# Chemical118/TREW

Hardware: NVIDIA B200
Metric: Gbases/s for trew short 5 32 at 1/2/4/8 B200; % of HBM roofline (higher is better)
Workload: dtype u64

## Files before the change

trew_b200/csrc/exact_thread.cuh:

```cuda
#pragma once
#include <stdint.h>

#if defined(__CUDACC__)
#define ET_HD __host__ __device__ __forceinline__
#define ET_FN __host__ __device__ __noinline__
#else
#define ET_HD inline
#define ET_FN inline
#endif
#if defined(__CUDA_ARCH__)
#define ET_UNROLL _Pragma("unroll")
#define ET_NO_UNROLL _Pragma("unroll 1")
#else
#define ET_UNROLL
#define ET_NO_UNROLL
#endif

namespace trew {
namespace et {

typedef uint32_t u32;
typedef uint64_t u64;
typedef unsigned __int128 u128;

// ... 13 lines not shown
    static constexpr int KW = (int)(sizeof(K) / 4);
    static constexpr int CT = W_CKEY + KW * kClsCap, WORDS = CT + kClsCap;
};
constexpr int kWorkWords = Lay<u64>::WORDS;

struct Mem {
    u32* base; int stride;
    ET_HD u32& operator[](int i) const { return base[i * stride]; }
};

ET_HD int popc(u32 x) {
#if defined(__CUDA_ARCH__)
    return __popc(x);
#else
    return __builtin_popcount(x);
#endif
}
ET_HD int ffs1(u32 x) {
#if defined(__CUDA_ARCH__)
    return __ffs(x) - 1;
#else
    return __builtin_ctz(x);
#endif
}
ET_HD u32 fshr(u32 lo, u32 hi, int sh) {
#if defined(__CUDA_ARCH__)
    return __funnelshift_r(lo, hi, sh);
#else
    sh &= 31;
    return sh ? (lo >> sh) | (hi << (32 - sh)) : lo;
#endif
}
ET_HD u32 brev32(u32 x) {
#if defined(__CUDA_ARCH__)
    return __brev(x);
#else
    x = ((x >> 1) & 0x55555555u) | ((x & 0x55555555u) << 1);
    x = ((x >> 2) & 0x33333333u) | ((x & 0x33333333u) << 2);
    x = ((x >> 4) & 0x0f0f0f0fu) | ((x & 0x0f0f0f0fu) << 4);
    x = ((x >> 8) & 0x00ff00ffu) | ((x & 0x00ff00ffu) << 8);
    return (x >> 16) | (x << 16);
#endif
}
ET_HD u32 lowmask(int bits) { return bits >= 32 ? 0xffffffffu : (bits <= 0 ? 0u : ((1u << bits) - 1u)); }
ET_HD u32 pxor32(u32 x) { x ^= x << 1; x ^= x << 2; x ^= x << 4; x ^= x << 8; x ^= x << 16; return x; }
ET_HD u64 spread(u32 x) {
    u64 v = x;
    v = (v | (v << 16)) & 0x0000FFFF0000FFFFULL;
    v = (v | (v << 8)) & 0x00FF00FF00FF00FFULL;
    v = (v | (v << 4)) & 0x0F0F0F0F0F0F0F0FULL;
    v = (v | (v << 2)) & 0x3333333333333333ULL;
    v = (v | (v << 1)) & 0x5555555555555555ULL;
    return v;
}

ET_FN u64 canon64(u64 w, int k) {
    const int sh = 2 * (k - 1);
    if (k <= 16) {
        u32 b = (u32)w, c = (u32)w;
        for (int r = 1; r < k; r++) { c = ((c & 3u) << sh) | (c >> 2); b = c < b ? c : b; }
        return b;
    }
    u64 best = w, cur = w;
    for (int r = 1; r < k; r++) { cur = ((cur & 3ULL) << sh) | (cur >> 2); best = cur < best ? cur : best; }
    return best;
}
ET_FN u128 canon128(u128 w, int k) {
    const int sh = 2 * (k - 1);
    u128 best = w, cur = w;
    for (int r = 1; r < k; r++) { cur = ((cur & 3) << sh) | (cur >> 2); best = cur < best ? cur : best; }
    return best;
}
ET_HD u64 canon(u64 w, int k) { return canon64(w, k); }
ET_HD u128 canon(u128 w, int k) { return k <= 32 ? (u128)canon64((u64)w, k) : canon128(w, k); }
ET_HD u64 crc(u64 w, int k) {
    const u32 lo = brev32((u32)w), hi = brev32((u32)(w >> 32));
    u64 x = ((u64)lo << 32) | hi;
    x = ((x >> 1) & 0x5555555555555555ULL) | ((x & 0x5555555555555555ULL) << 1);
    return canon64(~x >> (64 - 2 * k), k);
}
ET_HD u128 crc(u128 w, int k) {
    if (k <= 32) return (u128)crc((u64)w, k);
    u128 r = 0;
    for (int i = 0; i < k; i++) { r = (r << 2) | (3 - (w & 3)); w >>= 2; }
    return canon128(r, k);
}
ET_HD bool homo(u64 w, int k) {
    return k <= 1 || ((w ^ (w >> 2)) & ((1ULL << (2 * (k - 1))) - 1ULL)) == 0;
}
ET_HD bool homo(u128 w, int k) {
    return k <= 1 || ((w ^ (w >> 2)) & ((((u128)1) << (2 * (k - 1))) - 1)) == 0;
}

template <class K>
struct ClsSpill {
    K key[kClsSpill];
    unsigned short tot[kClsSpill], last[kClsSpill];
};

template <class K>
ET_HD K cls_key(Mem m, int q) {
    K v = 0;
    for (int i = Lay<K>::KW - 1; i >= 0; i--) v = (v << 16 << 16) | (K)m[W_CKEY + Lay<K>::KW * q + i];
    return v;
}
template <class K>
ET_HD void cls_put(Mem m, int q, K key) {
    for (int i = 0; i < Lay<K>::KW; i++) { m[W_CKEY + Lay<K>::KW * q + i] = (u32)key; key = key >> 16 >> 16; }
}

ET_HD u32 shr_plane(Mem m, int base, int j, int k) {
    if (k < 32) return fshr(m[base + j], m[base + j + 1], k);
    if (k == 32) return m[base + j + 1];
    if (k < 64) return fshr(m[base + j + 1], m[base + j + 2], k - 32);
    return m[base + j + 2];
}

ET_HD u64 raw_kmer(Mem m, int j, int b, int k, u64& hk, u64& lk, u64) {
    const u32 km = lowmask(k);
    const u32 h = fshr(m[W_H + j], m[W_H + j + 1], b) & km, l = fshr(m[W_L + j], m[W_L + j + 1], b) & km;
    hk = h; lk = l;
    return (spread(brev32(h) >> (32 - k)) << 1) | spread(brev32(l) >> (32 - k));
}
ET_HD u128 raw_kmer(Mem m, int j, int b, int k, u64& hk, u64& lk, u128) {
    if (k <= 32) return (u128)raw_kmer(m, j, b, k, hk, lk, (u64)0);
    const u64 km = k >= 64 ? ~0ULL : ((1ULL << k) - 1ULL);
    hk = ((u64)fshr(m[W_H + j], m[W_H + j + 1], b) | ((u64)fshr(m[W_H + j + 1], m[W_H + j + 2], b) << 32)) & km;
    lk = ((u64)fshr(m[W_L + j], m[W_L + j + 1], b) | ((u64)fshr(m[W_L + j + 1], m[W_L + j + 2], b) << 32)) & km;
    const u64 hr = (((u64)brev32((u32)hk) << 32) | brev32((u32)(hk >> 32))) >> (64 - k);
    const u64 lr = (((u64)brev32((u32)lk) << 32) | brev32((u32)(lk >> 32))) >> (64 - k);
    const u64 lo = (spread((u32)hr) << 1) | spread((u32)lr), hi = (spread((u32)(hr >> 32)) << 1) | spread((u32)(lr >> 32));
    return ((u128)hi << 64) | lo;
}

ET_HD u32 run_starts(Mem m, int j) {
    return m[W_WV + j] & ~((m[W_LINK + j] << 1) | (j ? m[W_LINK + j - 1] >> 31 : 0u));
}
ET_FN int prepare_runs(Mem m, int nw, int k) {
    for (int j = 0; j < nw; j++) {
        const u32 hs = shr_plane(m, W_H, j, k), ls = shr_plane(m, W_L, j, k);
        const u32 eq = ~((hs ^ m[W_H + j]) | (ls ^ m[W_L + j]));
        const u32 wvj = m[W_WV + j];
        const u32 nxt = (wvj >> 1) | (j + 1 < nw ? m[W_WV + j + 1] << 31 : 0u);
        m[W_LINK + j] = eq & wvj & nxt;
    }
    int runs = 0;
    for (int j = 0; j < nw; j++) runs += popc(run_starts(m, j));
    return runs;
}

constexpr int kMemo = 4;
#if defined(ET_MEMO_STATS) && !defined(__CUDA_ARCH__)
inline long memo_runs = 0, memo_hits = 0;
#define ET_MEMO_COUNT(hit) (memo_runs++, memo_hits += (hit) >= 0)
#else
#define ET_MEMO_COUNT(hit) ((void)0)
#endif
template <class K>
ET_FN int classify_runs(Mem m, int runs, int k, ClsSpill<K>& x, bool approx, int T = 0, int need_min = 0) {
    int n = 0, ord = 0, j = 0, best = 0;
    const int slack = T - need_min;
    K mraw[kMemo];
    u32 mcls = 0;
    int nm = 0;
    u32 wvj = m[W_WV], rr = run_starts(m, 0);
    for (int r = 0; r < runs; r++) {
        while (!rr) { ord += popc(wvj); j++; rr = run_starts(m, j); wvj = m[W_WV + j]; }
        {
            const int b = ffs1(rr);
            rr &= rr - 1;
            const u32 c0 = (u32)(ord + popc(wvj & ((1u << b) - 1u)));
            int jj = j;
            u32 z = ~m[W_LINK + j] & (0xffffffffu << b);
            while (!z) { jj++; z = ~m[W_LINK + jj]; }
            const u32 cnt = (u32)(32 * (jj - j) + ffs1(z) - b + 1);
            u64 hk, lk;
            const K raw = raw_kmer(m, j, b, k, hk, lk, (K)0);
            const u32 last = c0 + cnt - 1u;
            int hit = -1;
            if (!approx) {
ET_UNROLL
                for (int e = 0; e < kMemo; e++) hit = e < nm && mraw[e] == raw ? (int)((mcls >> (8 * e)) & 0xffu) : hit;
            }
            if (!approx) ET_MEMO_COUNT(hit);
            u32 tot = cnt;
            if (hit >= kClsCap) {
                const int s = hit - kClsCap;
                tot = x.tot[s] + cnt; x.tot[s] = (unsigned short)tot; x.last[s] = (unsigned short)last;
            } else if (hit >= 0) {
                const u32 ct = (m[Lay<K>::CT + hit] & 0xffff0000u) + (cnt << 16);
                m[Lay<K>::CT + hit] = ct | last;
                tot = ct >> 16;
            } else {
                K key;
                if (approx) key = (K)((u32)(popc((u32)hk) + popc((u32)(hk >> 32))) | ((u32)(popc((u32)lk) + popc((u32)(lk >> 32))) << 8) |
                                      ((u32)(popc((u32)(hk & lk)) + popc((u32)((hk & lk) >> 32))) << 16));
                else key = canon(raw, k);
                int q = 0;
                const int nq = n < kClsCap ? n : kClsCap;
                while (q < nq && cls_key<K>(m, q) != key) q++;
                if (q < nq) {
                    const u32 ct = (m[Lay<K>::CT + q] & 0xffff0000u) + (cnt << 16);
                    m[Lay<K>::CT + q] = ct | last;
                    tot = ct >> 16;
                } else if (n < kClsCap) {
                    cls_put<K>(m, n, key); m[Lay<K>::CT + n] = (cnt << 16) | last;
                    n++;
                } else {
                    int s = 0;
                    while (s < n - kClsCap && x.key[s] != key) s++;
                    if (s < n - kClsCap) { tot = x.tot[s] + cnt; x.tot[s] = (unsigned short)tot; x.last[s] = (unsigned short)last; }
                    else { x.key[s] = key; x.tot[s] = (unsigned short)cnt; x.last[s] = (unsigned short)last; n++; }
                    q = kClsCap + s;
                }
                if (!approx && nm < kMemo) {
ET_UNROLL
                    for (int e = 0; e < kMemo; e++) if (e == nm) mraw[e] = raw;
                    mcls |= (u32)q << (8 * nm);
                    nm++;
                }
            }
            if (need_min > 0) {
                best = (int)tot > best ? (int)tot : best;
                if ((int)last + 1 - best > slack) return -1;
            }
        }
    }
    return n;
}

template <class K>
ET_FN int cls_max(Mem m, int n, const ClsSpill<K>& x, K& S) {
    u32 best = 0;
    S = 0;
    for (int q = 0; q < n && q < kClsCap; q++) {
        const u32 ct = m[Lay<K>::CT + q];
        const u32 score = ((ct >> 16) << 10) | (1023u - (ct & 0xffffu));
        if (score > best) { best = score; S = cls_key<K>(m, q); }
    }
    for (int q = 0; q < n - kClsCap; q++) {
        const u32 score = ((u32)x.tot[q] << 10) | (1023u - x.last[q]);
        if (score > best) { best = score; S = x.key[q]; }
    }
    return (int)(best >> 10);
}

ET_HD bool need_pass(const unsigned short* thr, u32 need, int M, int T) {
    const u32 mm = need & 0xffffu, t = need >> 16;
    return M >= (int)thr[T] && (t == 0u || (u32)M * t >= mm * (u32)T);
}

ET_HD int min_accept(const unsigned short* thr, u32 need, int T) {
    const u32 mm = need & 0xffffu, t = need >> 16;
    const int a = (int)thr[T], b = t ? (int)((mm * (u32)T + t - 1u) / t) : 0;
    return a > b ? a : b;
}

ET_HD void shrink_valid(Mem m, int nw) {
    for (int j = 0; j < nw; j++) m[W_WV + j] &= (m[W_WV + j] >> 1) | (j + 1 < nw ? m[W_WV + j + 1] << 31 : 0u);
}

template <int NW>
ET_HD void shrink_valid(u32 (&wv)[NW]) {
ET_UNROLL
    for (int j = 0; j < NW; j++) wv[j] &= (wv[j] >> 1) | (j + 1 < NW ? wv[j + 1] << 31 : 0u);
}
template <int S, int NW>
ET_HD void sig_counts(const u32 (&ph)[NW + 2], const u32 (&pl)[NW + 2], const u32 (&wv)[NW], int k, int& cH, int& cL, int& c11) {
ET_UNROLL
    for (int j = 0; j < NW; j++) {
        const u32 dh = (fshr(ph[S + j], S + j + 1 < NW + 2 ? ph[S + j + 1] : 0u, k) ^ ph[j]) & wv[j];
        const u32 dl = (fshr(pl[S + j], S + j + 1 < NW + 2 ? pl[S + j + 1] : 0u, k) ^ pl[j]) & wv[j];
        cH += popc(dh); cL += popc(dl); c11 += popc(dh & dl);
    }
}

template <class K> struct PeriodSet { typedef u64 T; };
template <> struct PeriodSet<u64> { typedef u32 T; };

template <class K, int NW>
ET_HD u32 scan_periods(Mem m, int len, int kmin, int kmax, const unsigned short* thr_low, const unsigned short* thr_high, ClsSpill<K>& x,
                       K (&S)[2]) {
    const int nw = (len + 31) >> 5;
    u32 ph[NW + 2], pl[NW + 2], wv[NW];
    {
        u32 ch = 0, cl = 0, tph = 0, tpl = 0;
ET_UNROLL
        for (int j = 0; j <= NW; j++) {
            const u32 ih = pxor32(m[W_H + j]) ^ ch, il = pxor32(m[W_L + j]) ^ cl;
            ph[j] = (ih << 1) | tph; pl[j] = (il << 1) | tpl;
            tph = ih >> 31; tpl = il >> 31;
            ch = 0u - tph; cl = 0u - tpl;
        }
        ph[NW + 1] = 0u; pl[NW + 1] = 0u;
    }
ET_UNROLL
    for (int j = 0; j < NW; j++) wv[j] = j < nw ? m[W_V + j] : 0u;
    for (int t = 1; t < kmin; t++) shrink_valid<NW>(wv);
    typedef typename PeriodSet<K>::T Set;
    Set blockedL = 0, blockedH = 0;
    u32 needL = 0, needH = 0;
    u32 res = 0;
ET_NO_UNROLL
    for (int k = kmin; k <= kmax; k++, shrink_valid<NW>(wv)) {
        const bool blkL = (bool)((blockedL >> (k - 1)) & 1u), blkH = (bool)((blockedH >> (k - 1)) & 1u);
        int T = 0, cH = 0, cL = 0, c11 = 0;
ET_UNROLL
        for (int j = 0; j < NW; j++) T += popc(wv[j]);
        if (T == 0) break;
        if (blkL && blkH) continue;
        if (k < 32) sig_counts<0, NW>(ph, pl, wv, k, cH, cL, c11);
        else if constexpr (sizeof(K) == 8) sig_counts<1, NW>(ph, pl, wv, k, cH, cL, c11);
        else if (k < 64) sig_counts<1, NW>(ph, pl, wv, k, cH, cL, c11);
        else sig_counts<2, NW>(ph, pl, wv, k, cH, cL, c11);
        const int c10 = cH - c11, c01 = cL - c11, c00 = T - cH - cL + c11;
        int U = c00 > c01 ? c00 : c01;
        U = U > c10 ? U : c10;
        U = U > c11 ? U : c11;
        if (!((!blkL && need_pass(thr_low, needL, U, T)) || (!blkH && need_pass(thr_high, needH, U, T)))) continue;
        K Sk;
ET_UNROLL
        for (int j = 0; j < NW; j++) m[W_WV + j] = wv[j];
        const int runs = prepare_runs(m, nw, k);
        int need_min = 1 << 20;
        if (!blkL) need_min = min_accept(thr_low, needL, T);
        if (!blkH) { const int a = min_accept(thr_high, needH, T); need_min = a < need_min ? a : need_min; }
        if (runs > 3 && T <= kApproxMaxWindows) {
            const int na = classify_runs(m, runs, k, x, true, T, need_min);
            if (na < 0) continue;
            const int Mu = cls_max(m, na, x, Sk);
            if (!((!blkL && need_pass(thr_low, needL, Mu, T)) || (!blkH && need_pass(thr_high, needH, Mu, T)))) continue;
        }
        const int n = classify_runs(m, runs, k, x, false, T, need_min);
        if (n < 0) continue;
        const int M = cls_max(m, n, x, Sk);
        if (homo(Sk, k)) continue;
        const bool accL = !blkL && need_pass(thr_low, needL, M, T), accH = !blkH && need_pass(thr_high, needH, M, T);
        if (accL || accH) {
            Set mm = 0;
            for (int j = k; j <= kmax; j += k) mm |= ((Set)1) << (j - 1);
            const u32 need = (u32)M | ((u32)T << 16);
            if (accL) { res = (res & 0xffu) | ((u32)k << 8); needL = need; blockedL |= mm; S[1] = Sk; }
            if (accH) { res = (res & 0xff00u) | (u32)k; needH = need; blockedH |= mm; S[0] = Sk; }
        }
    }
    return res;
}
template <class K>
ET_FN u32 scan_window(Mem m, int len, int kmin, int kmax, const unsigned short* thr_low, const unsigned short* thr_high, ClsSpill<K>& x,
                      K (&S)[2]) {
    S[0] = S[1] = 0;
    if (kmax > len) kmax = len;
    if (kmax < kmin) return 0u;
    if (len <= 96) return scan_periods<K, 3>(m, len, kmin, kmax, thr_low, thr_high, x, S);
    return scan_periods<K, kReadWords>(m, len, kmin, kmax, thr_low, thr_high, x, S);
}

enum { T_F = 0, T_B = 2, T_O = 4 };

template <class K, class Emit>
ET_HD void emit_window_classes(Mem m, int len, int k, int table, bool folded, ClsSpill<K>& x, Emit& emit);

template <class K, class Load, class Emit>
ET_HD bool route_short_thread(Mem m, int n, u32 pm, int min_mer, int max_mer, const unsigned short* thr_low,
                              const unsigned short* thr_high, Load& load, Emit& emit) {
    if (n < 2 * min_mer) return true;
    if (max_mer > (int)(4 * sizeof(K)) || n > kMaxRead) return false;
    const int kmax = n / 4 < max_mer ? n / 4 : max_mer;
    const int llen = n / 2, rlen = (n + 1) / 2, roff = n - rlen;
    ClsSpill<K> x;
    u32 L = 0, R = 0;
    K S[2];
    const bool halves = n >= 4 * min_mer;
    for (u32 todo = halves ? pm & 3u : 0u; todo != 0u; todo &= todo - 1u) {
        const bool right = (todo & 1u) == 0u;
        const int len = right ? rlen : llen;
        load(0, right ? roff : 0, len);
        const u32 r = scan_window(m, len, min_mer, kmax, thr_low, thr_high, x, S);
        if (right) R = r; else L = r;
    }
    if (4 * max_mer > n) {
        const bool hc0 = ((L | R) & 0xffu) == 0u, hc1 = ((L | R) >> 8) == 0u;
        const u32 wbit = halves ? 4u : 1u;
        if ((hc0 || hc1) && (pm & wbit)) {
            const int lo = n / 4 + 1 > min_mer ? n / 4 + 1 : min_mer, hi = n / 2 < max_mer ? n / 2 : max_mer;
            load(0, 0, n);
            const u32 W = scan_window(m, n, lo, hi, thr_low, thr_high, x, S);
            for (int c = 0; c < 2; c++) {
                const int k = (int)((W >> (8 * c)) & 0xffu);
                if ((c == 0 ? hc0 : hc1) && k) emit_window_classes(m, n, k, T_O + c, false, x, emit);
            }
        }
    }
    if ((L | R) == 0u) return true;
    int cur_win = -1, cur_k = 0, ncls = 0, T = 0;
    for (int c = 0; c < 2; c++) {
        const int Lc = (int)((L >> (8 * c)) & 0xffu), Rc = (int)((R >> (8 * c)) & 0xffu);
        int win, k, table;
        if (Lc > 0 && Lc == Rc) { win = 2; k = Lc; table = T_O + c; }
        else if (Lc > 0) { win = 0; k = Lc; table = T_F + c; }
        else if (Rc > 0) { win = 1; k = Rc; table = T_B + c; }
        else continue;
        if (win != cur_win || k != cur_k) {
            const int off = win == 1 ? roff : 0, len = win == 2 ? n : (win == 0 ? llen : rlen), nw = (len + 31) >> 5;
            load(0, off, len);
            for (int j = 0; j < nw; j++) m[W_WV + j] = m[W_V + j];
            for (int t = 1; t < k; t++) shrink_valid(m, nw);
            T = 0;
            for (int j = 0; j < nw; j++) T += popc(m[W_WV + j]);
            ncls = 0;
            if (T) ncls = classify_runs(m, prepare_runs(m, nw, k), k, x, false);
            cur_win = win; cur_k = k;
        }
        if (T == 0) continue;
        const bool target = win == 2;
        if (target) {
            K S;
            const int M = cls_max(m, ncls, x, S);
            if (homo(S, k) || M < (int)(c == 0 ? thr_high : thr_low)[T]) continue;
        }
        for (int q = 0; q < ncls; q++) {
            K key = q < kClsCap ? cls_key<K>(m, q) : x.key[q - kClsCap];
            const u64 cnt = q < kClsCap ? (u64)(m[Lay<K>::CT + q] >> 16) : (u64)x.tot[q - kClsCap];
            if (target) { const K t = crc(key, k); key = t < key ? t : key; }
            emit(table, k, key, cnt);
        }
    }
    return true;
}

template <class K, class Emit>
ET_HD void emit_window_classes(Mem m, int len, int k, int table, bool folded, ClsSpill<K>& x, Emit& emit) {
    const int nw = (len + 31) >> 5;
    for (int j = 0; j < nw; j++) m[W_WV + j] = m[W_V + j];
    for (int t = 1; t < k; t++) shrink_valid(m, nw);
    int T = 0;
    for (int j = 0; j < nw; j++) T += popc(m[W_WV + j]);
    if (T == 0) return;
    const int ncls = classify_runs(m, prepare_runs(m, nw, k), k, x, false);
    for (int q = 0; q < ncls; q++) {
        K key = q < kClsCap ? cls_key<K>(m, q) : x.key[q - kClsCap];
        const u64 cnt = q < kClsCap ? (u64)(m[Lay<K>::CT + q] >> 16) : (u64)x.tot[q - kClsCap];
        if (folded) { const K t = crc(key, k); key = t < key ? t : key; }
        emit(table, k, key, cnt);
    }
}

template <class K, class Load, class Emit>
ET_HD bool route_pair_thread(Mem m, int n1, int n2, int min_mer, int max_mer, const unsigned short* thr_low,
                             const unsigned short* thr_high, Load& load, Emit& emit) {
    const int n = n1 < n2 ? n1 : n2;
    if (n < 2 * min_mer) return true;
    if (max_mer > (int)(4 * sizeof(K)) || n1 > kMaxRead || n2 > kMaxRead || 4 * max_mer > n) return false;
    const int kmax = n / 4 < max_mer ? n / 4 : max_mer;
    const int soff[5] = {0, 0, n1 - (n1 + 1) / 2, n2 - (n2 + 1) / 2, 0};
    const int slen[5] = {0, n1 / 2, (n1 + 1) / 2, (n2 + 1) / 2, n2 / 2};
    ClsSpill<K> x;
    u32 res[5] = {0, 0, 0, 0, 0};
    K S[5][2];
    bool have[5] = {false, false, false, false, false};
    auto window = [&](int t) { load(t <= 2 ? 0 : 1, soff[t], slen[t]); };
    auto scan = [&](int t) {
        if (have[t]) return;
        window(t);
        res[t] = scan_window(m, slen[t], min_mer, kmax, thr_low, thr_high, x, S[t]);
        have[t] = true;
    };
    int pseg[2][8], ptmp[2][8], np[2] = {0, 0};
    int si[2] = {1, 1}, km[2] = {0, 0};
    bool ended[2] = {false, false};
    K ks[2] = {0, 0};
    for (int ti = 1; ti <= 4 && !(ended[0] && ended[1]); ti++) {
        scan(ti);
        for (int c = 0; c < 2; c++) {
            const int k = (int)((res[ti] >> (8 * c)) & 0xffu);
            if (!ended[c] && k) { pseg[c][np[c]] = ti; ptmp[c][np[c]] = ti <= 2 ? 0 : 1; np[c]++; }
            bool ok = !ended[c] && k > 0;
            if (ok && ti != 1) {
                const K ds = ti > 2 ? crc(S[ti][c], k) : S[ti][c];
                ok = km[c] == k && ks[c] == ds;
            }
            if (ok) { si[c]++; km[c] = k; if (ti == 1) ks[c] = S[ti][c]; }
            else ended[c] = true;
        }
    }
    for (int c = 0; c < 2; c++) {
        if (si[c] == 5) {
            for (int e = 0; e < np[c]; e++) {
                const int sg = pseg[c][e];
                window(sg);
                emit_window_classes(m, slen[sg], (int)((res[sg] >> (8 * c)) & 0xffu), T_O + c, true, x, emit);
            }
        }
    }
    if (si[0] <= 4 || si[1] <= 4) {
        int sj[2] = {4, 4};
        km[0] = km[1] = 0; ended[0] = ended[1] = false;
        for (int tj = 4; tj >= 1 && !(ended[0] && ended[1]); tj--) {
            scan(tj);
            for (int c = 0; c < 2; c++) {
                const int k = (int)((res[tj] >> (8 * c)) & 0xffu);
                if (!ended[c] && k) { pseg[c][np[c]] = tj; ptmp[c][np[c]] = tj <= 2 ? 1 : 0; np[c]++; }
                bool ok = sj[c] >= si[c] && !ended[c] && k > 0;
                if (ok && tj != 4) {
                    const K ds = tj <= 2 ? crc(S[tj][c], k) : S[tj][c];
                    ok = km[c] == k && ks[c] == ds;
                }
                if (ok) { sj[c]--; km[c] = k; if (tj == 4) ks[c] = S[tj][c]; }
                else ended[c] = true;
            }
        }
    }
    for (int c = 0; c < 2; c++) {
        if (si[c] <= 4) {
            for (int e = 0; e < np[c]; e++) {
                const int sg = pseg[c][e];
                window(sg);
                emit_window_classes(m, slen[sg], (int)((res[sg] >> (8 * c)) & 0xffu), (ptmp[c][e] == 0 ? T_F : T_B) + c, false, x, emit);
            }
        }
    }
    return true;
}


struct LongGeom {
    int n, SL, snum, mid, bonus;
    ET_HD LongGeom(int n_, int SL_) : n(n_), SL(SL_), snum(n_ / SL_), mid((n_ / SL_ + 1) / 2), bonus(n_ % SL_) {}
    ET_HD int start(int t) const { return (t - 1) * SL + (t > mid ? bonus : 0); }
    ET_HD int len(int t) const { return SL + (t == mid ? bonus : 0); }
};

template <class Load>
ET_HD u32 long_slice_stats(Mem m, const LongGeom& g, int t, int min_mer, int max_mer, const unsigned short* thr_low,
                           const unsigned short* thr_high, Load& load, ClsSpill<u64>& x) {
    const int len = g.len(t);
    load(0, g.start(t), len);
    u64 S[2];
    return scan_window(m, len, min_mer, max_mer, thr_low, thr_high, x, S);
}

struct LongTask { unsigned short slice; unsigned char k, table_folded; };

template <class Stat, class Task>
ET_HD bool long_walk(const LongGeom& g, Stat& stat, Task& task) {
    const int snum = g.snum;
    const bool mid_ok = g.len(g.mid) <= kMaxRead;
    for (int pass = mid_ok ? 1 : 0; pass < 2; pass++) {
        int si[2] = {1, 1}, km[2] = {0, 0};
        bool ended[2] = {false, false};
        int nf = 0;
        for (int ti = 1; ti <= snum && !(ended[0] && ended[1]); ti++) {
            if (pass == 0 && ti == g.mid) return false;
            const u32 r = stat(ti);
            for (int c = 0; c < 2; c++) {
                const int k = (int)((r >> (8 * c)) & 0xffu);
                if (!ended[c] && k > 0 && (ti == 1 || km[c] == k)) { si[c]++; km[c] = k; }
                else ended[c] = true;
            }
            nf = ti;
        }
        if (pass == 1) {
            bool en[2] = {false, false};
            int kk[2] = {0, 0};
            const bool full[2] = {si[0] == snum + 1, si[1] == snum + 1};
            for (int ti = 1; ti <= nf; ti++) {
                const u32 r = stat(ti);
                for (int c = 0; c < 2; c++) {
                    const int k = (int)((r >> (8 * c)) & 0xffu);
                    if (!en[c] && k) task(LongTask{(unsigned short)ti, (unsigned char)k, (unsigned char)(((full[c] ? T_O : T_F) + c) | (full[c] ? 8 : 0))});
                    if (!en[c] && k > 0 && (ti == 1 || kk[c] == k)) kk[c] = k;
                    else en[c] = true;
                }
            }
        }
        if (si[0] <= snum || si[1] <= snum) {
            int sj[2] = {snum, snum};
            km[0] = km[1] = 0; ended[0] = ended[1] = false;
            for (int tj = snum; tj >= 1 && !(ended[0] && ended[1]); tj--) {
                if (pass == 0 && tj == g.mid) return false;
// ... 23 lines not shown
```

trew_b200/csrc/scan_kernels.cu:

```cuda
#include "scan_kernels.cuh"
#include "exact_thread.cuh"

#include <cstdio>

namespace trew {

typedef unsigned int u32;
typedef unsigned long long u64;
typedef unsigned __int128 u128;


__device__ __forceinline__ u32 lane_id() { return threadIdx.x & 31; }

__device__ __forceinline__ u32 low_mask(int bits) {
    return bits >= 32 ? 0xffffffffu : ((1u << bits) - 1u);
}

__device__ __forceinline__ u32 prefix_xor32(u32 x) {
    x ^= x << 1; x ^= x << 2; x ^= x << 4; x ^= x << 8; x ^= x << 16;
    return x;
}

__device__ __forceinline__ u64 mix64(u64 x) {
    x ^= x >> 33; x *= 0xff51afd7ed558ccdULL; x ^= x >> 33; x *= 0xc4ceb9fe1a85ec53ULL; x ^= x >> 33;
// ... 1440 lines not shown
                if (!have[tj]) { sr[tj] = scan_stats(ws, b, spos[tj], slen[tj], MINM, kmax, cfg); have[tj] = true; }
                int k[2] = {sr[tj].th, sr[tj].tl};
                u64 slo[2] = {sr[tj].sh_lo, sr[tj].sl_lo}, shi[2] = {sr[tj].sh_hi, sr[tj].sl_hi};
#pragma unroll
                for (int c = 0; c < 2; c++) {
                    if (!ended[c] && k[c]) { pseg[c][np[c]] = tj; ptmp[c][np[c]] = tj <= 2 ? 1 : 0; np[c]++; }
                    bool ok = sj[c] >= si[c] && !ended[c] && k[c] > 0;
                    if (ok && tj != 4) {
                        u64 dlo = slo[c], dhi = shi[c];
                        if (tj <= 2) crc_pair(dlo, dhi, k[c]);
                        ok = km[c] == k[c] && ks_lo[c] == dlo && ks_hi[c] == dhi;
                    }
                    if (ok) { sj[c]--; km[c] = k[c]; if (tj == 4) { ks_lo[c] = slo[c]; ks_hi[c] = shi[c]; } }
                    else ended[c] = true;
                }
            }
        }
#pragma unroll
        for (int c = 0; c < 2; c++) {
            if (si[c] <= 4) {
                for (int e = 0; e < np[c]; e++) {
                    int sg = pseg[c][e];
                    emit_window(tr, ws, b, spos[sg], slen[sg], c == 0 ? sr[sg].th : sr[sg].tl,
                                (ptmp[c][e] == 0 ? T_F : T_B) + c, false);
                }
            }
        }
    }
    if (4 * MAXM > n && (lef[0] == 0 || lef[1] == 0 || km[0] == 0 || km[1] == 0)) {
        int lo = max(n / 4 + 1, MINM), hi = min(n / 2, MAXM);
        ScanRes l, r; l.th = l.tl = r.th = r.tl = 0; l.sh_lo = l.sh_hi = l.sl_lo = l.sl_hi = 0; r = l;
        if (lef[0] == 0 || lef[1] == 0) l = scan_stats(ws, b, a0, n1, lo, hi, cfg);
        if (km[0] == 0 || km[1] == 0) r = scan_stats(ws, b, a1, n2, lo, hi, cfg);
        int ltk[2] = {l.th, l.tl}, rtk[2] = {r.th, r.tl};
        u64 llo[2] = {l.sh_lo, l.sl_lo}, lhi[2] = {l.sh_hi, l.sl_hi}, rlo[2] = {r.sh_lo, r.sl_lo}, rhi[2] = {r.sh_hi, r.sl_hi};
#pragma unroll
        for (int c = 0; c < 2; c++) {
            bool el = lef[c] == 0 && ltk[c] > 0, er = km[c] == 0 && rtk[c] > 0;
            bool both = lef[c] == 0 && km[c] == 0 && ltk[c] == rtk[c] && ltk[c] > 0;
            if (both) {
                u64 dlo = rlo[c], dhi = rhi[c];
                crc_pair(dlo, dhi, rtk[c]);
                both = llo[c] == dlo && lhi[c] == dhi;
            }
            if (both) {
                if (el) emit_window(tr, ws, b, a0, n1, ltk[c], T_O + c, true);
                if (er) emit_window(tr, ws, b, a1, n2, rtk[c], T_O + c, true);
            }
            if (el) emit_window(tr, ws, b, a0, n1, ltk[c], T_F + c, false);
            if (er) emit_window(tr, ws, b, a1, n2, rtk[c], T_F + c, false);
        }
    }
}

__device__ void route_long(const DevCfg& cfg, TableRef tr, WS ws, const DevBatch& b, u32 u, unsigned char* scratch) {
    const int MINM = cfg.min_mer, MAXM = cfg.max_mer, SL = cfg.slice_len;
    u32 b0 = __ldg(b.bit_off + u);
    int n = (int)(__ldg(b.bit_off + u + 1) - b0);
    if (n < SL) return;
    int snum = n / SL, mid = (snum + 1) / 2, bonus = n % SL;
    auto s_start = [&](int t) { return (u32)((t - 1) * SL + (t > mid ? bonus : 0)); };
    auto s_len = [&](int t) { return SL + (t == mid ? bonus : 0); };
    int si[2] = {1, 1}, km[2] = {0, 0}; bool ended[2] = {false, false};
    int nf = 0;
    for (int ti = 1; ti <= snum && !(ended[0] && ended[1]); ti++) {
        ScanRes sr = scan_stats(ws, b, b0 + s_start(ti), s_len(ti), MINM, MAXM, cfg);
        if (ws.lane == 0) { scratch[2 * (ti - 1)] = (unsigned char)sr.th; scratch[2 * (ti - 1) + 1] = (unsigned char)sr.tl; }
        int k[2] = {sr.th, sr.tl};
#pragma unroll
        for (int c = 0; c < 2; c++) {
            if (!ended[c] && k[c] > 0 && (ti == 1 || km[c] == k[c])) { si[c]++; km[c] = k[c]; }
            else ended[c] = true;
        }
        nf = ti;
    }
    __syncwarp();
    {
        bool en[2] = {false, false}; int kk[2] = {0, 0};
        bool full[2] = {si[0] == snum + 1, si[1] == snum + 1};
        for (int ti = 1; ti <= nf; ti++) {
            int k[2] = {scratch[2 * (ti - 1)], scratch[2 * (ti - 1) + 1]};
#pragma unroll
            for (int c = 0; c < 2; c++) {
                if (!en[c] && k[c]) emit_window(tr, ws, b, b0 + s_start(ti), s_len(ti), k[c], (full[c] ? T_O : T_F) + c, full[c]);
                if (!en[c] && k[c] > 0 && (ti == 1 || kk[c] == k[c])) kk[c] = k[c];
                else en[c] = true;
            }
        }
    }
    if (si[0] <= snum || si[1] <= snum) {
        int sj[2] = {snum, snum}; km[0] = km[1] = 0; ended[0] = ended[1] = false;
        for (int tj = snum; tj >= 1 && !(ended[0] && ended[1]); tj--) {
            ScanRes sr = scan_stats(ws, b, b0 + s_start(tj), s_len(tj), MINM, MAXM, cfg);
            int k[2] = {sr.th, sr.tl};
#pragma unroll
            for (int c = 0; c < 2; c++) {
                if (!ended[c] && k[c]) emit_window(tr, ws, b, b0 + s_start(tj), s_len(tj), k[c], T_B + c, false);
                if (sj[c] >= si[c] && !ended[c] && k[c] > 0 && (tj == snum || km[c] == k[c])) { sj[c]--; km[c] = k[c]; }
                else ended[c] = true;
            }
        }
    }
}


constexpr int kStageSlots = 256;
constexpr int kStageProbes = 6;
constexpr u32 kStageLock = 0xffffffffu;

struct StageEmit {
    u32* s_meta; u32* s_cnt; u64* s_key;
    Slot* slots; u32 mask; u32* err;
    __device__ __forceinline__ void operator()(int table, int k, et::u128 key, u64 count) const {
        const u64 hi = (u64)(key >> 64);
        if (hi) table_add_impl(slots, mask, err, ((u32)table << 8) | (u32)k, (u64)key, hi, count);
        else (*this)(table, k, (et::u64)key, count);
    }
    __device__ __forceinline__ void operator()(int table, int k, et::u64 key_, u64 count) const {
        const u64 key = (u64)key_;
        const u32 meta = ((u32)table << 8) | (u32)k, tag = meta | 0x80000000u;
        u32 i = (u32)(mix64(key ^ ((u64)meta << 53)) >> 40) & (kStageSlots - 1);
        bool done = false;
        for (int p = 0; p < kStageProbes && !done; p++, i = (i + 1) & (kStageSlots - 1)) {
            int outcome = 0;
            do {
                const u32 st = atomicCAS(&s_meta[i], 0u, kStageLock);
                if (st == 0u) {
                    s_key[i] = key;
                    __threadfence_block();
                    atomicExch(&s_meta[i], tag);
                    atomicAdd(&s_cnt[i], (u32)count);
                    outcome = 1;
                } else if (st != kStageLock) {
                    __threadfence_block();
                    if (st == tag && *(volatile u64*)&s_key[i] == key) { atomicAdd(&s_cnt[i], (u32)count); outcome = 1; }
                    else outcome = 2;
                }
            } while (outcome == 0);
            done = outcome == 1;
        }
        if (!done) table_add_impl(slots, mask, err, meta, key, 0ULL, count);
    }
};

#ifndef TREW_THREAD_BLOCK
#define TREW_THREAD_BLOCK 128
#endif
template <class K>
constexpr size_t thread_kernel_smem() { return (size_t)et::Lay<K>::WORDS * TREW_THREAD_BLOCK * sizeof(u32) + (size_t)kStageSlots * 16; }
constexpr size_t kThreadKernelSmem = thread_kernel_smem<et::u64>();
template <int MODE, class K>
constexpr int thread_kernel_bps() { return (sizeof(K) == 8 ? 6 : 5) - (MODE == 1 ? 1 : 0); }

struct PlaneLoad {
    et::Mem m; const u32 *hi, *lo, *val; u32 b0[2];
    __device__ __forceinline__ void operator()(int mate, int off, int len) const {
        const u32 pos = b0[mate] + (u32)off, w0 = pos >> 5, sh = pos & 31u;
        for (int j = 0; j < et::kReadWords + 2; j++) {
            const u32 msk = low_mask(min(32, max(0, len - 32 * j)));
            u32 h = 0u, l = 0u;
            if (msk) {
                h = __funnelshift_r(__ldg(hi + w0 + j), __ldg(hi + w0 + j + 1), sh) & msk;
                l = __funnelshift_r(__ldg(lo + w0 + j), __ldg(lo + w0 + j + 1), sh) & msk;
            }
            m[et::W_H + j] = h; m[et::W_L + j] = l;
            if (j < et::kReadWords) m[et::W_V + j] = msk ? __funnelshift_r(__ldg(val + w0 + j), __ldg(val + w0 + j + 1), sh) & msk : 0u;
        }
    }
};

template <int MODE, class K>
__global__ void __launch_bounds__(TREW_THREAD_BLOCK, (thread_kernel_bps<MODE, K>())) trew_exact_thread_kernel(DevCfg cfg, DevBatch b, const u32* __restrict__ survivors,
                                                                              const u32* __restrict__ n_survivors, int packed_probes,
                                                                              u32* __restrict__ hard, u32* __restrict__ n_hard,
                                                                              unsigned long long* total_survivors, u32* work_counter) {
    u32* work = reinterpret_cast<u32*>(g_smem);
    u64* s_key = reinterpret_cast<u64*>(work + et::Lay<K>::WORDS * TREW_THREAD_BLOCK);
    u32* s_meta = reinterpret_cast<u32*>(s_key + kStageSlots);
    u32* s_cnt = s_meta + kStageSlots;
    for (int i = threadIdx.x; i < kStageSlots; i += blockDim.x) { s_meta[i] = 0u; s_cnt[i] = 0u; }
    __syncthreads();
    const et::Mem m{work + threadIdx.x, TREW_THREAD_BLOCK};
    const u32 n = *n_survivors;
    if (blockIdx.x == 0 && threadIdx.x == 0 && total_survivors) atomicAdd(total_survivors, (unsigned long long)n);
    StageEmit emit{s_meta, s_cnt, s_key, cfg.slots, cfg.slot_mask, cfg.error_flag};
    for (;;) {
        u32 base = 0;
        if (lane_id() == 0) base = atomicAdd(work_counter, 32u);
        base = __shfl_sync(0xffffffffu, base, 0);
        if (base >= n) break;
        const u32 i = base + lane_id();
        bool bail = false;
        u32 entry = 0;
        if (i < n) {
            entry = survivors[i];
            u32 u = entry, pm = 3u;
            if (packed_probes) { pm = entry >> kProbeShift; u &= (1u << kProbeShift) - 1u; }
            if (MODE == 0) {
                const u32 b0 = __ldg(b.bit_off + u);
                const int len = (int)(__ldg(b.bit_off + u + 1) - b0);
                if (len > et::kMaxRead) {
                    bail = true;
                } else {
                    PlaneLoad load{m, b.hi, b.lo, b.val, {b0, 0u}};
                    bail = !et::route_short_thread<K>(m, len, pm & 7u, cfg.min_mer, cfg.max_mer, cfg.thr_low, cfg.thr_high, load, emit);
                }
            } else {
                const u32 a0 = __ldg(b.bit_off + 2 * u), a1 = __ldg(b.bit_off + 2 * u + 1), a2 = __ldg(b.bit_off + 2 * u + 2);
                const int n1 = (int)(a1 - a0), n2 = (int)(a2 - a1);
                PlaneLoad load{m, b.hi, b.lo, b.val, {a0, a1}};
                bail = !et::route_pair_thread<K>(m, n1, n2, cfg.min_mer, cfg.max_mer, cfg.thr_low, cfg.thr_high, load, emit);
            }
        }
        list_append(bail, entry, hard, n_hard);
    }
    __syncthreads();
    for (int i = threadIdx.x; i < kStageSlots; i += blockDim.x) {
        const u32 st = s_meta[i], c = s_cnt[i];
        if (st != 0u && st != kStageLock && c != 0u) table_add_impl(cfg.slots, cfg.slot_mask, cfg.error_flag, st & 0x7fffffffu, s_key[i], 0ULL, (u64)c);
    }
}


struct LongArgs {
    const u32* survivors; const u32* n_survivors; int packed_probes;
    u32 s_cap, max_slices;
    unsigned short* stats; u32* emis;
    u32* hard; u32* n_hard;
    unsigned long long* total_survivors;
};

__global__ void __launch_bounds__(TREW_THREAD_BLOCK, 4) trew_long_stats_kernel(DevCfg cfg, DevBatch b, LongArgs a) {
    u32* work = reinterpret_cast<u32*>(g_smem);
    const et::Mem m{work + threadIdx.x, TREW_THREAD_BLOCK};
    const u32 n = min(*a.n_survivors, a.s_cap);
    const u32 warps = gridDim.x * (blockDim.x >> 5), lane = lane_id();
    et::ClsSpill<et::u64> x;
    for (u32 idx = blockIdx.x * (blockDim.x >> 5) + (threadIdx.x >> 5); idx < n; idx += warps) {
        u32 u = a.survivors[idx];
        if (a.packed_probes) u &= (1u << kProbeShift) - 1u;
        const u32 b0 = __ldg(b.bit_off + u);
        const int len = (int)(__ldg(b.bit_off + u + 1) - b0);
        if (len < cfg.slice_len) continue;
        const et::LongGeom g(len, cfg.slice_len);
        PlaneLoad load{m, b.hi, b.lo, b.val, {b0, 0u}};
        unsigned short* row = a.stats + (size_t)idx * (a.max_slices + 1);
        for (int t = 1 + (int)lane; t <= g.snum; t += 32) {
            u32 r = 0;
            if (g.len(t) <= et::kMaxRead) r = et::long_slice_stats(m, g, t, cfg.min_mer, cfg.max_mer, cfg.thr_low, cfg.thr_high, load, x);
            row[t] = (unsigned short)r;
        }
    }
}

__global__ void __launch_bounds__(256) trew_long_walk_kernel(DevCfg cfg, DevBatch b, LongArgs a) {
    const u32 n_all = *a.n_survivors;
    if (blockIdx.x == 0 && threadIdx.x == 0 && a.total_survivors) atomicAdd(a.total_survivors, (unsigned long long)n_all);
    const u32 stride = gridDim.x * blockDim.x, n_round = (n_all + 31u) & ~31u;
    for (u32 idx = blockIdx.x * blockDim.x + threadIdx.x; idx < n_round; idx += stride) {
        bool bail = false;
        u32 entry = 0;
        if (idx < n_all) {
            entry = a.survivors[idx];
            u32 u = entry;
            if (a.packed_probes) u &= (1u << kProbeShift) - 1u;
            const int len = (int)(__ldg(b.bit_off + u + 1) - __ldg(b.bit_off + u));
            if (idx >= a.s_cap) bail = len >= cfg.slice_len;
            else if (len >= cfg.slice_len) {
                const et::LongGeom g(len, cfg.slice_len);
                const unsigned short* row = a.stats + (size_t)idx * (a.max_slices + 1);
                u32* em = a.emis + (size_t)idx * (a.max_slices + 1);
                for (int t = 1; t <= g.snum; t++) em[t] = 0u;
                auto stat = [&](int t) { return (u32)row[t]; };
                auto task = [&](const et::LongTask& tk) {
                    const int tb = tk.table_folded & 7, c = tb & 1;
                    const bool backward = (tb & 6) == et::T_B;
                    const u32 byte = (u32)tk.k | ((tk.table_folded & 8) ? 0x80u : 0u);
                    em[tk.slice] |= byte << (8 * ((backward ? 2 : 0) + c));
                };
                bail = !et::long_walk(g, stat, task);
                if (bail) for (int t = 1; t <= g.snum; t++) em[t] = 0u;
            }
        }
        list_append(bail, entry, a.hard, a.n_hard);
    }
}

__global__ void __launch_bounds__(TREW_THREAD_BLOCK, 4) trew_long_emit_kernel(DevCfg cfg, DevBatch b, LongArgs a) {
    u32* work = reinterpret_cast<u32*>(g_smem);
    u64* s_key = reinterpret_cast<u64*>(work + et::Lay<et::u64>::WORDS * TREW_THREAD_BLOCK);
    u32* s_meta = reinterpret_cast<u32*>(s_key + kStageSlots);
    u32* s_cnt = s_meta + kStageSlots;
    for (int i = threadIdx.x; i < kStageSlots; i += blockDim.x) { s_meta[i] = 0u; s_cnt[i] = 0u; }
    __syncthreads();
    const et::Mem m{work + threadIdx.x, TREW_THREAD_BLOCK};
    StageEmit emit{s_meta, s_cnt, s_key, cfg.slots, cfg.slot_mask, cfg.error_flag};
    const u32 n = min(*a.n_survivors, a.s_cap);
    const u32 warps = gridDim.x * (blockDim.x >> 5), lane = lane_id();
    et::ClsSpill<et::u64> x;
    for (u32 idx = blockIdx.x * (blockDim.x >> 5) + (threadIdx.x >> 5); idx < n; idx += warps) {
        u32 u = a.survivors[idx];
        if (a.packed_probes) u &= (1u << kProbeShift) - 1u;
        const u32 b0 = __ldg(b.bit_off + u);
        const int len = (int)(__ldg(b.bit_off + u + 1) - b0);
        if (len < cfg.slice_len) continue;
        const et::LongGeom g(len, cfg.slice_len);
        PlaneLoad load{m, b.hi, b.lo, b.val, {b0, 0u}};
        const u32* em = a.emis + (size_t)idx * (a.max_slices + 1);
        for (int t = 1 + (int)lane; t <= g.snum; t += 32) {
            const u32 e = em[t];
            if (e == 0u) continue;
            for (int f = 0; f < 4; f++) {
                const u32 byte = (e >> (8 * f)) & 0xffu;
                if (byte == 0u) continue;
                const int c = f & 1;
                const bool folded = (byte & 0x80u) != 0u;
                const int table = (f >= 2 ? et::T_B : (folded ? et::T_O : et::T_F)) + c;
                et::LongTask tk{(unsigned short)t, (unsigned char)(byte & 0x7fu), (unsigned char)(table | (folded ? 8 : 0))};
                et::long_emit(m, g, tk, load, x, emit);
            }
        }
    }
    __syncthreads();
    for (int i = threadIdx.x; i < kStageSlots; i += blockDim.x) {
        const u32 st = s_meta[i], c = s_cnt[i];
        if (st != 0u && st != kStageLock && c != 0u) table_add_impl(cfg.slots, cfg.slot_mask, cfg.error_flag, st & 0x7fffffffu, s_key[i], 0ULL, (u64)c);
    }
}

bool long_thread_path_applies(const DevCfg& cfg) { return cfg.mode == 2 && cfg.max_mer <= 32 && cfg.slice_len <= et::kMaxRead; }

size_t long_thread_scratch_bytes(unsigned int s_cap, unsigned int max_slices) {
    return (size_t)s_cap * (max_slices + 1) * (sizeof(unsigned short) + sizeof(u32)) + 64;
}

void launch_long_thread(const DevCfg& cfg, const DevBatch& b, const unsigned int* survivors, const unsigned int* n_survivors,
                        int packed_probes, unsigned int s_cap, unsigned int max_slices, unsigned char* scratch, unsigned int* hard,
                        unsigned int* n_hard, unsigned long long* total_survivors, int sm_count, cudaStream_t stream) {
    LongArgs a{};
    a.survivors = survivors; a.n_survivors = n_survivors; a.packed_probes = packed_probes;
    a.s_cap = s_cap; a.max_slices = max_slices;
    a.emis = reinterpret_cast<u32*>(scratch);
    a.stats = reinterpret_cast<unsigned short*>(scratch + (size_t)s_cap * (max_slices + 1) * sizeof(u32));
    a.hard = hard; a.n_hard = n_hard; a.total_survivors = total_survivors;
    const size_t smem_stats = (size_t)et::Lay<et::u64>::WORDS * TREW_THREAD_BLOCK * sizeof(u32);
    trew_long_stats_kernel<<<sm_count * 4, TREW_THREAD_BLOCK, smem_stats, stream>>>(cfg, b, a);
    trew_long_walk_kernel<<<sm_count * 2, 256, 0, stream>>>(cfg, b, a);
    trew_long_emit_kernel<<<sm_count * 4, TREW_THREAD_BLOCK, kThreadKernelSmem, stream>>>(cfg, b, a);
}

bool thread_path_applies(const DevCfg& cfg, unsigned int max_read_len) {
    if (cfg.max_mer > 64) return false;
    if (cfg.mode == 0) return true;
    return cfg.mode == 1 && max_read_len >= 4u * (unsigned)cfg.max_mer;
}

void launch_exact_thread(const DevCfg& cfg, const DevBatch& b, const unsigned int* survivors, const unsigned int* n_survivors,
                         int packed_probes, unsigned int* hard, unsigned int* n_hard, unsigned long long* total_survivors, int sm_count,
                         int blocks_per_sm, unsigned int* work_counter, cudaStream_t stream) {
    const bool wide = cfg.max_mer > 32;
#define TREW_LAUNCH_THREAD(MODE, K)                                                                                               \
    trew_exact_thread_kernel<MODE, K><<<sm_count * (blocks_per_sm > 0 ? blocks_per_sm : thread_kernel_bps<MODE, K>()),            \
                                        TREW_THREAD_BLOCK, thread_kernel_smem<K>(), stream>>>(                                    \
        cfg, b, survivors, n_survivors, packed_probes, hard, n_hard, total_survivors, work_counter)
    if (cfg.mode == 0) { if (wide) TREW_LAUNCH_THREAD(0, et::u128); else TREW_LAUNCH_THREAD(0, et::u64); }
    else               { if (wide) TREW_LAUNCH_THREAD(1, et::u128); else TREW_LAUNCH_THREAD(1, et::u64); }
#undef TREW_LAUNCH_THREAD
// ... 57 lines not shown
```

Measured before the change: 1035.

## Park short reads needing emit phase and process them in full warps

Splits the short-read routine into a resumable state machine (half scans, whole scan, emit). In the MODE 0 thread kernel, reads that reach the emit phase are parked in per-warp shared memory slots and drained 32 at a time, so the costly classify/emit step runs with a fully converged warp. The goal is less branch divergence, where a few lanes doing emit work would otherwise stall the rest of the warp. In exchange it adds shared memory use, a reload of the read planes when emitting, and ballot/sync overhead.

```diff
diff --git a/trew_b200/csrc/exact_thread.cuh b/trew_b200/csrc/exact_thread.cuh
--- a/trew_b200/csrc/exact_thread.cuh
+++ b/trew_b200/csrc/exact_thread.cuh
@@ -189,9 +189,12 @@
 constexpr int kMemo = 4;
 #if defined(ET_MEMO_STATS) && !defined(__CUDA_ARCH__)
 inline long memo_runs = 0, memo_hits = 0;
+inline long cost_iters = 0, cost_runs = 0;
 #define ET_MEMO_COUNT(hit) (memo_runs++, memo_hits += (hit) >= 0)
+#define ET_COST(counter) (counter++)
 #else
 #define ET_MEMO_COUNT(hit) ((void)0)
+#define ET_COST(counter) ((void)0)
 #endif
 template <class K>
 ET_FN int classify_runs(Mem m, int runs, int k, ClsSpill<K>& x, bool approx, int T = 0, int need_min = 0) {
@@ -202,6 +205,7 @@
     int nm = 0;
     u32 wvj = m[W_WV], rr = run_starts(m, 0);
     for (int r = 0; r < runs; r++) {
+        ET_COST(cost_runs);
         while (!rr) { ord += popc(wvj); j++; rr = run_starts(m, j); wvj = m[W_WV + j]; }
         {
             const int b = ffs1(rr);
@@ -340,6 +344,7 @@
     u32 res = 0;
 ET_NO_UNROLL
     for (int k = kmin; k <= kmax; k++, shrink_valid<NW>(wv)) {
+        ET_COST(cost_iters);
         const bool blkL = (bool)((blockedL >> (k - 1)) & 1u), blkH = (bool)((blockedH >> (k - 1)) & 1u);
         int T = 0, cH = 0, cL = 0, c11 = 0;
 ET_UNROLL
@@ -398,38 +403,62 @@
 template <class K, class Emit>
 ET_HD void emit_window_classes(Mem m, int len, int k, int table, bool folded, ClsSpill<K>& x, Emit& emit);
 
+enum { SR_HALF = 0, SR_WHOLE = 1, SR_EMIT = 2 };
+struct ShortRead {
+    int n;
+    u32 todo;
+    u32 L, R;
+    int phase;
+};
+
+ET_HD int short_next(ShortRead& s, int max_mer) {
+    if (s.phase == SR_HALF && (s.todo & 3u)) return 0;
+    if (s.phase == SR_HALF) {
+        const bool hc0 = ((s.L | s.R) & 0xffu) == 0u, hc1 = ((s.L | s.R) >> 8) == 0u;
+        s.phase = SR_WHOLE;
+        if (4 * max_mer > s.n && (hc0 || hc1) && (s.todo & 4u)) return 0;
+    }
+    if (s.phase == SR_WHOLE && (s.L | s.R) != 0u) { s.phase = SR_EMIT; return 0; }
+    return 1;
+}
+
+template <class K>
+ET_HD int short_begin(ShortRead& s, int n, u32 pm, int min_mer, int max_mer) {
+    if (n < 2 * min_mer) return 1;
+    if (max_mer > (int)(4 * sizeof(K)) || n > kMaxRead) return -1;
+    s.n = n;
+    s.todo = n >= 4 * min_mer ? pm & 7u : (pm & 1u) << 2;
+    s.L = s.R = 0u;
+    s.phase = SR_HALF;
+    return short_next(s, max_mer);
+}
+
 template <class K, class Load, class Emit>
-ET_HD bool route_short_thread(Mem m, int n, u32 pm, int min_mer, int max_mer, const unsigned short* thr_low,
-                              const unsigned short* thr_high, Load& load, Emit& emit) {
-    if (n < 2 * min_mer) return true;
-    if (max_mer > (int)(4 * sizeof(K)) || n > kMaxRead) return false;
-    const int kmax = n / 4 < max_mer ? n / 4 : max_mer;
+ET_HD int short_step(Mem m, ShortRead& s, int min_mer, int max_mer, const unsigned short* thr_low, const unsigned short* thr_high,
+                     Load& load, Emit& emit) {
+    const int n = s.n;
     const int llen = n / 2, rlen = (n + 1) / 2, roff = n - rlen;
     ClsSpill<K> x;
-    u32 L = 0, R = 0;
-    K S[2];
-    const bool halves = n >= 4 * min_mer;
-    for (u32 todo = halves ? pm & 3u : 0u; todo != 0u; todo &= todo - 1u) {
-        const bool right = (todo & 1u) == 0u;
-        const int len = right ? rlen : llen;
-        load(0, right ? roff : 0, len);
-        const u32 r = scan_window(m, len, min_mer, kmax, thr_low, thr_high, x, S);
-        if (right) R = r; else L = r;
-    }
-    if (4 * max_mer > n) {
-        const bool hc0 = ((L | R) & 0xffu) == 0u, hc1 = ((L | R) >> 8) == 0u;
-        const u32 wbit = halves ? 4u : 1u;
-        if ((hc0 || hc1) && (pm & wbit)) {
-            const int lo = n / 4 + 1 > min_mer ? n / 4 + 1 : min_mer, hi = n / 2 < max_mer ? n / 2 : max_mer;
-            load(0, 0, n);
-            const u32 W = scan_window(m, n, lo, hi, thr_low, thr_high, x, S);
+    if (s.phase != SR_EMIT) {
+        const bool whole = s.phase == SR_WHOLE, right = !whole && (s.todo & 1u) == 0u;
+        const int off = right ? roff : 0, len = whole ? n : (right ? rlen : llen);
+        const int lo = whole && n / 4 + 1 > min_mer ? n / 4 + 1 : min_mer;
+        const int hi = whole ? (n / 2 < max_mer ? n / 2 : max_mer) : (n / 4 < max_mer ? n / 4 : max_mer);
+        K S[2];
+        load(0, off, len);
+        const u32 r = scan_window(m, len, lo, hi, thr_low, thr_high, x, S);
+        if (!whole) {
+            if (right) s.R = r; else s.L = r;
+            s.todo &= s.todo - 1u;
+        } else {
             for (int c = 0; c < 2; c++) {
-                const int k = (int)((W >> (8 * c)) & 0xffu);
-                if ((c == 0 ? hc0 : hc1) && k) emit_window_classes(m, n, k, T_O + c, false, x, emit);
-            }
-        }
-    }
-    if ((L | R) == 0u) return true;
+                const int k = (int)((r >> (8 * c)) & 0xffu);
+                if (((s.L | s.R) >> (8 * c) & 0xffu) == 0u && k) emit_window_classes(m, n, k, T_O + c, false, x, emit);
+            }
+        }
+        return short_next(s, max_mer);
+    }
+    const u32 L = s.L, R = s.R;
     int cur_win = -1, cur_k = 0, ncls = 0, T = 0;
     for (int c = 0; c < 2; c++) {
         const int Lc = (int)((L >> (8 * c)) & 0xffu), Rc = (int)((R >> (8 * c)) & 0xffu);
@@ -463,6 +492,16 @@
             emit(table, k, key, cnt);
         }
     }
+    return 1;
+}
+
+template <class K, class Load, class Emit>
+ET_HD bool route_short_thread(Mem m, int n, u32 pm, int min_mer, int max_mer, const unsigned short* thr_low,
+                              const unsigned short* thr_high, Load& load, Emit& emit) {
+    ShortRead s;
+    const int st = short_begin<K>(s, n, pm, min_mer, max_mer);
+    if (st != 0) return st > 0;
+    while (!short_step<K>(m, s, min_mer, max_mer, thr_low, thr_high, load, emit)) {}
     return true;
 }
 
diff --git a/trew_b200/csrc/scan_kernels.cu b/trew_b200/csrc/scan_kernels.cu
--- a/trew_b200/csrc/scan_kernels.cu
+++ b/trew_b200/csrc/scan_kernels.cu
@@ -1616,6 +1616,8 @@
 template <int MODE, class K>
 constexpr int thread_kernel_bps() { return (sizeof(K) == 8 ? 6 : 5) - (MODE == 1 ? 1 : 0); }
 
+constexpr u32 kParkSlots = 64;
+
 struct PlaneLoad {
     et::Mem m; const u32 *hi, *lo, *val; u32 b0[2];
     __device__ __forceinline__ void operator()(int mate, int off, int len) const {
@@ -1648,35 +1650,79 @@
     const u32 n = *n_survivors;
     if (blockIdx.x == 0 && threadIdx.x == 0 && total_survivors) atomicAdd(total_survivors, (unsigned long long)n);
     StageEmit emit{s_meta, s_cnt, s_key, cfg.slots, cfg.slot_mask, cfg.error_flag};
-    for (;;) {
-        u32 base = 0;
-        if (lane_id() == 0) base = atomicAdd(work_counter, 32u);
-        base = __shfl_sync(0xffffffffu, base, 0);
-        if (base >= n) break;
-        const u32 i = base + lane_id();
-        bool bail = false;
-        u32 entry = 0;
-        if (i < n) {
-            entry = survivors[i];
-            u32 u = entry, pm = 3u;
-            if (packed_probes) { pm = entry >> kProbeShift; u &= (1u << kProbeShift) - 1u; }
-            if (MODE == 0) {
-                const u32 b0 = __ldg(b.bit_off + u);
+    if constexpr (MODE == 0) {
+        __shared__ u32 s_park[3 * kParkSlots * (TREW_THREAD_BLOCK / 32)];
+        u32* park_b0 = s_park + 3 * kParkSlots * (threadIdx.x >> 5);
+        u32* park_n = park_b0 + kParkSlots;
+        u32* park_lr = park_n + kParkSlots;
+        const u32 lane = lane_id();
+        u32 parked = 0;
+        auto emit_parked = [&](u32 cnt) {
+            if (lane < cnt) {
+                const u32 slot = parked - cnt + lane;
+                et::ShortRead sr;
+                sr.n = (int)park_n[slot]; sr.todo = 0u; sr.L = park_lr[slot] & 0xffffu; sr.R = park_lr[slot] >> 16; sr.phase = et::SR_EMIT;
+                PlaneLoad load{m, b.hi, b.lo, b.val, {park_b0[slot], 0u}};
+                et::short_step<K>(m, sr, cfg.min_mer, cfg.max_mer, cfg.thr_low, cfg.thr_high, load, emit);
+            }
+            __syncwarp();
+            parked -= cnt;
+        };
+        for (;;) {
+            u32 base = 0;
+            if (lane == 0) base = atomicAdd(work_counter, 32u);
+            base = __shfl_sync(0xffffffffu, base, 0);
+            if (base >= n) break;
+            const u32 i = base + lane;
+            bool bail = false, park = false;
+            u32 entry = 0, b0 = 0;
+            et::ShortRead sr;
+            if (i < n) {
+                entry = survivors[i];
+                u32 u = entry, pm = 3u;
+                if (packed_probes) { pm = entry >> kProbeShift; u &= (1u << kProbeShift) - 1u; }
+                b0 = __ldg(b.bit_off + u);
                 const int len = (int)(__ldg(b.bit_off + u + 1) - b0);
-                if (len > et::kMaxRead) {
-                    bail = true;
-                } else {
+                const int st = len > et::kMaxRead ? -1 : et::short_begin<K>(sr, len, pm & 7u, cfg.min_mer, cfg.max_mer);
+                bail = st < 0;
+                if (st == 0) {
                     PlaneLoad load{m, b.hi, b.lo, b.val, {b0, 0u}};
-                    bail = !et::route_short_thread<K>(m, len, pm & 7u, cfg.min_mer, cfg.max_mer, cfg.thr_low, cfg.thr_high, load, emit);
+                    int done = 0;
+                    while (!done && sr.phase != et::SR_EMIT) done = et::short_step<K>(m, sr, cfg.min_mer, cfg.max_mer, cfg.thr_low, cfg.thr_high, load, emit);
+                    park = !done;
                 }
-            } else {
+            }
+            list_append(bail, entry, hard, n_hard);
+            const u32 pk = __ballot_sync(0xffffffffu, park);
+            if (park) {
+                const u32 slot = parked + (u32)__popc(pk & ((1u << lane) - 1u));
+                park_b0[slot] = b0; park_n[slot] = (u32)sr.n; park_lr[slot] = sr.L | (sr.R << 16);
+            }
+            __syncwarp();
+            parked += (u32)__popc(pk);
+            if (parked >= 32u) emit_parked(32u);
+        }
+        if (parked) emit_parked(parked);
+    } else {
+        for (;;) {
+            u32 base = 0;
+            if (lane_id() == 0) base = atomicAdd(work_counter, 32u);
+            base = __shfl_sync(0xffffffffu, base, 0);
+            if (base >= n) break;
+            const u32 i = base + lane_id();
+            bool bail = false;
+            u32 entry = 0;
+            if (i < n) {
+                entry = survivors[i];
+                u32 u = entry;
+                if (packed_probes) u &= (1u << kProbeShift) - 1u;
                 const u32 a0 = __ldg(b.bit_off + 2 * u), a1 = __ldg(b.bit_off + 2 * u + 1), a2 = __ldg(b.bit_off + 2 * u + 2);
                 const int n1 = (int)(a1 - a0), n2 = (int)(a2 - a1);
                 PlaneLoad load{m, b.hi, b.lo, b.val, {a0, a1}};
                 bail = !et::route_pair_thread<K>(m, n1, n2, cfg.min_mer, cfg.max_mer, cfg.thr_low, cfg.thr_high, load, emit);
             }
-        }
-        list_append(bail, entry, hard, n_hard);
+            list_append(bail, entry, hard, n_hard);
+        }
     }
     __syncthreads();
     for (int i = threadIdx.x; i < kStageSlots; i += blockDim.x) {
```

Measured after the change: 1021 (median of 6 runs). 0.987x the previous value.
